# sizhe-li/neural-jacobian-field

Hardware: AMD Instinct MI355X
Metric: rendered rays/s (64 samples/ray, 256^2 image) (higher is better)
Workload: dtype f32 (v_mfma_f32_32x32x2_f32: exact fp32 products, fp32 accumulate -- the reference's arithmetic)

## Files before the change

neural-jacobian-field_amd/csrc/njf_device.h:

```cpp
#pragma once
#include <hip/hip_runtime.h>
#include <stdint.h>

__device__ __forceinline__ float relu_bits(float x) { return __int_as_float(max(__float_as_int(x), 0)); }

typedef float f32x16 __attribute__((ext_vector_type(16)));
typedef float f32x4 __attribute__((ext_vector_type(4)));
typedef _Float16 f16x8 __attribute__((ext_vector_type(8)));
typedef _Float16 f16x16 __attribute__((ext_vector_type(16)));
typedef _Float16 f16x32 __attribute__((ext_vector_type(32)));
typedef int i32x8 __attribute__((ext_vector_type(8)));
typedef int i32x4 __attribute__((ext_vector_type(4)));
typedef int i32x2 __attribute__((ext_vector_type(2)));
typedef unsigned u32x6 __attribute__((ext_vector_type(6)));

#define PREC_F32 0
#define PREC_F16X2 1
#define PREC_F16F6 2
#define PREC_F16 3

#define NJF_WAVES 4
#define NJF_THREADS (NJF_WAVES * 64)
#define NJF_CHUNK 8192

#define NJF_STREAM_BUFFERS 2
#define LDS_CTR_FLOATS 0
#define LDS_W0 0
#define LDS_W1 NJF_CHUNK
#define LDS_BIAS (NJF_STREAM_BUFFERS * NJF_CHUNK)
#define LDS_BIAS_FLOATS 2752
#define LDS_BIAS_FLOATS_PROPOSAL 1344
#define LDS_SCRATCH_PER_WAVE 528
#define LDS_FLOATS_RENDER (LDS_BIAS + LDS_BIAS_FLOATS + LDS_CTR_FLOATS)
#define LDS_FLOATS_PROPOSAL (LDS_BIAS + LDS_BIAS_FLOATS_PROPOSAL + NJF_WAVES * LDS_SCRATCH_PER_WAVE + LDS_CTR_FLOATS)
#define LDS_SCRATCH_PROPOSAL (LDS_BIAS + LDS_BIAS_FLOATS_PROPOSAL)

extern __shared__ __attribute__((aligned(16))) float njf_lds[];

__device__ __forceinline__ float mfma_step(float a, float b, f32x16& c) {
  c = __builtin_amdgcn_mfma_f32_32x32x2f32(a, b, c, 0, 0, 0);
  return 0.f;
}

#ifdef NJF_STAMPS
#define NJF_STAMP_SLOTS 1024
#ifdef NJF_STAMPS_PROPOSAL
#define NJF_STAMP_BASE LDS_FLOATS_PROPOSAL
#define NJF_STAMP_LOGS_PROPOSAL true
#else
#define NJF_STAMP_BASE LDS_FLOATS_RENDER
#define NJF_STAMP_LOGS_PROPOSAL false
#endif
__device__ unsigned njf_stamp_out[NJF_STAMP_SLOTS];
#define NJF_STAMP_FIELD int stamp_i;
#define NJF_STAMP_INIT(st) (st).stamp_i = -1
#define NJF_STAMP(st, tag)                                                                                   \
  do {                                                                                                       \
    if ((st).stamp_i >= 0 && (st).stamp_i < NJF_STAMP_SLOTS) {                                               \
      njf_lds[NJF_STAMP_BASE + (st).stamp_i] =                                                               \
          __uint_as_float(((unsigned)(tag) << 24) | ((unsigned)__builtin_readcyclecounter() & 0xffffffu));   \
      (st).stamp_i += 1;                                                                                     \
    }                                                                                                        \
  } while (0)
#define NJF_STAMP_P(st, tag) do { if (NJF_STAMP_LOGS_PROPOSAL) NJF_STAMP(st, tag); } while (0)
#define NJF_STAMP_ARM(st, IS_PROPOSAL, wave)                                                                                \
  const bool njf_stamping = ((IS_PROPOSAL) == NJF_STAMP_LOGS_PROPOSAL) && blockIdx.x == gridDim.x / 2 + 3 && (wave) == 1; \
  if (njf_stamping) (st).stamp_i = 0;                                                                                     \
  NJF_STAMP(st, 9)
#define NJF_STAMP_FLUSH(st, tag, lane)                                                                       \
  do {                                                                                                       \
    NJF_STAMP(st, tag);                                                                                      \
    if (njf_stamping)                                                                                        \
      for (int i_ = (lane); i_ < NJF_STAMP_SLOTS; i_ += 64)                                                  \
        njf_stamp_out[i_] = i_ < (st).stamp_i ? __float_as_uint(njf_lds[NJF_STAMP_BASE + i_]) : 0u;          \
  } while (0)
#define NJF_STAMP_PIN(...) asm volatile("" : __VA_ARGS__)
#define NJF_STAMP_LDS_FLOATS NJF_STAMP_SLOTS
#else
#define NJF_STAMP_FIELD
#define NJF_STAMP_INIT(st) do {} while (0)
#define NJF_STAMP(st, tag) do {} while (0)
#define NJF_STAMP_P(st, tag) do {} while (0)
#define NJF_STAMP_ARM(st, IS_PROPOSAL, wave) do {} while (0)
#define NJF_STAMP_FLUSH(st, tag, lane) do {} while (0)
#define NJF_STAMP_PIN(...) do {} while (0)
#define NJF_STAMP_LDS_FLOATS 0
#endif

struct WeightStreamState {
  __amdgpu_buffer_rsrc_t rsrc;
  int per_pass;
  int total;
  int idx;
  int in_pass;
  int dma_voff;
  int dma_soff;
  float* dma_dst;
  int dma_next;
  NJF_STAMP_FIELD
};
template <int GAP_AT_, int GAP_>
struct WeightStreamT : WeightStreamState {
  static constexpr int GAP_AT = GAP_AT_, GAP = GAP_;
};
typedef WeightStreamT<0x7fffffff, 0> WeightStream;
#define NJF_DMA_ROUNDS (NJF_CHUNK / (NJF_THREADS * 4))

__device__ __forceinline__ void dma_issue(const WeightStreamState& st, int r) {
#ifdef NJF_ABLATE_DMA
  return;
#endif
  __builtin_amdgcn_raw_ptr_buffer_load_lds(st.rsrc, (__attribute__((address_space(3))) void*)(st.dma_dst + r * NJF_THREADS * 4),
                                           16, st.dma_voff, st.dma_soff + r * NJF_THREADS * 16, 0, 0);
}

__device__ __forceinline__ void stream_flush(WeightStreamState& st) {
  if (st.dma_next == 0) {
#pragma unroll
    for (int r = 0; r < NJF_DMA_ROUNDS; ++r) dma_issue(st, r);
    st.dma_next = NJF_DMA_ROUNDS;
  }
}

template <class ST>
__device__ __forceinline__ void dma_job(ST& st, int chunk, int buf, int wave) {
  if constexpr (ST::GAP != 0) {
    if (chunk >= ST::GAP_AT) chunk += ST::GAP;
  }
  st.dma_soff = chunk * (NJF_CHUNK * 4) + wave * 1024;
  st.dma_dst = njf_lds + buf * NJF_CHUNK + wave * 256;
  st.dma_next = 0;
}

template <class ST>
__device__ __forceinline__ void stream_begin(ST& st, const float* g, int per_pass, int passes, int wave,
                                             int lane) {
  st.rsrc = __builtin_amdgcn_make_buffer_rsrc((void*)g, 0, 0x7ffffff0, 0x00020000);
  st.per_pass = per_pass;
  st.total = per_pass * passes;
  st.idx = 0;
  st.in_pass = 0;
  st.dma_voff = lane * 16;
  NJF_STAMP_INIT(st);
  dma_job(st, 0, 0, wave);
  stream_flush(st);
}

template <class ST>
__device__ __forceinline__ const float* stream_step(ST& st, int wave, int lane) {
#ifdef NJF_ABLATE_BARRIER
  return njf_lds + (st.idx++ & 1) * NJF_CHUNK;
#endif
  stream_flush(st);
  NJF_STAMP(st, 1);
  asm volatile("s_waitcnt vmcnt(0)" ::: "memory");
  NJF_STAMP(st, 2);
  __syncthreads();
  NJF_STAMP(st, 3);
  const float* cur = njf_lds + (st.idx & 1) * NJF_CHUNK;
  st.idx += 1;
  st.in_pass += 1;
  if (st.in_pass == st.per_pass) st.in_pass = 0;
  if (st.idx < st.total) dma_job(st, st.in_pass, st.idx & 1, wave);
  return cur;
}


typedef _Float16 f16x2 __attribute__((ext_vector_type(2)));
typedef unsigned u32x4 __attribute__((ext_vector_type(4)));
template <bool RELU>
__device__ __forceinline__ void split_pair(float x0, float x1, int p, f16x8& hi, f16x8& lo) {
  if (RELU) {
    x0 = relu_bits(x0);
    x1 = relu_bits(x1);
  }
  const _Float16 h0 = (_Float16)x0, h1 = (_Float16)x1;
  hi[2 * p] = h0;
  hi[2 * p + 1] = h1;
  const f16x2 hp = {h0, h1};
  const unsigned hu = __builtin_bit_cast(unsigned, hp);
  unsigned lu;
  asm("v_fma_mixlo_f16 %0, -%1, 1.0, %2 op_sel:[0,0,0] op_sel_hi:[1,0,0]" : "=v"(lu) : "v"(hu), "v"(x0));
  asm("v_fma_mixhi_f16 %0, -%1, 1.0, %2 op_sel:[1,0,0] op_sel_hi:[1,0,0]" : "+v"(lu) : "v"(hu), "v"(x1));
  u32x4 lv = __builtin_bit_cast(u32x4, lo);
  lv[p] = lu;
  lo = __builtin_bit_cast(f16x8, lv);
}

typedef unsigned u32x16 __attribute__((ext_vector_type(16)));
__device__ __forceinline__ unsigned pk_max_u16(unsigned a, unsigned b) {
  unsigned r;
  asm("v_pk_max_u16 %0, %1, %2" : "=v"(r) : "v"(a), "v"(b));
  return r;
}
template <bool RELU>
__device__ __forceinline__ void split_pair_u(float x0, float x1, unsigned& hu, unsigned& lu) {
  if (RELU) {
    x0 = relu_bits(x0);
    x1 = relu_bits(x1);
  }
  const f16x2 hp = {(_Float16)x0, (_Float16)x1};
  hu = __builtin_bit_cast(unsigned, hp);
  asm("v_fma_mixlo_f16 %0, -%1, 1.0, %2 op_sel:[0,0,0] op_sel_hi:[1,0,0]" : "=v"(lu) : "v"(hu), "v"(x0));
  asm("v_fma_mixhi_f16 %0, -%1, 1.0, %2 op_sel:[1,0,0] op_sel_hi:[1,0,0]" : "+v"(lu) : "v"(hu), "v"(x1));
}

typedef short s16x2 __attribute__((ext_vector_type(2)));
template <bool RELU>
__device__ __forceinline__ unsigned pack_pair_f16(float x0, float x1) {
  typedef float f32x2 __attribute__((ext_vector_type(2)));
  const f32x2 xp = {x0, x1};
  const f16x2 hp = __builtin_convertvector(xp, f16x2);
  if constexpr (RELU) {
    const s16x2 z = {0, 0};
    return __builtin_bit_cast(unsigned, __builtin_elementwise_max(__builtin_bit_cast(s16x2, hp), z));
  } else {
    return __builtin_bit_cast(unsigned, hp);
  }
}

#define F6_HI 0
#define F6_P1 16384
#define F6_P2 24576
#define F6_SCALE 28672


template <int PREC, int MBO, int NKB, int KB0, bool RELU, int KBI, class ST>
__device__ __forceinline__ void mma_chunk(ST& st, const float* __restrict__ wl, int lane,
                                          const f32x16 (&in)[KBI], f32x16 (&out)[MBO]) {
  constexpr bool SPREAD = MBO == 4 && (NKB == 2 || (PREC == PREC_F16 && NKB == 4)) && NJF_DMA_ROUNDS == 8;
  if constexpr (!SPREAD) stream_flush(st);
  if constexpr (PREC == PREC_F32) {
    const float* base = wl + lane * 4;
#pragma unroll
    for (int kb = 0; kb < NKB; ++kb) {
#pragma unroll
      for (int q = 0; q < 4; ++q) {
        f32x4 a[MBO];
#pragma unroll
        for (int m = 0; m < MBO; ++m) a[m] = *(const f32x4*)(base + ((kb * 4 + q) * MBO + m) * 256);
        if constexpr (SPREAD) {
          if (kb * 4 + q < 4) {
            dma_issue(st, 2 * (kb * 4 + q));
            dma_issue(st, 2 * (kb * 4 + q) + 1);
          }
        }
#pragma unroll
        for (int e = 0; e < 4; ++e) {
          float b = in[KB0 + kb][q * 4 + e];
          if (RELU) b = relu_bits(b);
#pragma unroll
          for (int m = 0; m < MBO; ++m) out[m] = __builtin_amdgcn_mfma_f32_32x32x2f32(a[m][e], b, out[m], 0, 0, 0);
        }
      }
    }
  } else if constexpr (PREC == PREC_F16F6 && MBO == 4 && NKB == 2) {
    typedef __attribute__((address_space(3))) const char* lds_ptr;
    const lds_ptr wb = (lds_ptr)(const char*)wl;
    lds_ptr p16 = wb + lane * 16;
    lds_ptr p8 = wb + lane * 8;
    asm volatile("" : "+v"(p16), "+v"(p8));
    unsigned bh[4][4], bl[4][4], mx[4];
#pragma unroll
    for (int p = 0; p < 4; ++p) {
      split_pair_u<RELU>(in[KB0][2 * p], in[KB0][2 * p + 1], bh[0][p], bl[0][p]);
      mx[p] = RELU ? bh[0][p] : (bh[0][p] & 0x7fff7fffu);
    }
#define NJF_LDS(T) const __attribute__((address_space(3))) T*
    auto hfrag = [&](int i) { return *(NJF_LDS(f16x8))(p16 + i * 1024); };
    auto f6frag = [&](int idx) {
      const i32x4 a4 = *(NJF_LDS(i32x4))(p16 + F6_P1 + idx * 1024);
      const i32x2 b2 = *(volatile NJF_LDS(i32x2))(p8 + F6_P2 + idx * 512);
      return i32x8{a4[0], a4[1], a4[2], a4[3], b2[0], b2[1], 0, 0};
    };
    auto op8 = [](const unsigned (&v)[4]) { return __builtin_bit_cast(f16x8, u32x4{v[0], v[1], v[2], v[3]}); };
    f16x8 a[2] = {hfrag(0), hfrag(1)};
    unsigned sb_h = 0, sb_l = 0;
    i32x8 bh6 = {0, 0, 0, 0, 0, 0, 0, 0}, wl6_0 = bh6, wl6_1 = bh6;
#pragma unroll
    for (int t = 0; t < 4; ++t) {
#pragma unroll
      for (int half = 0; half < 2; ++half) {
        const int u = 2 * t + half;
        f16x8 n[2] = {a[0], a[1]};
        if (u + 1 < 8) {
          n[0] = hfrag((u + 1) * 2);
          n[1] = hfrag((u + 1) * 2 + 1);
        } else {
          wl6_0 = f6frag(1);
          wl6_1 = f6frag(3);
        }
        if constexpr (SPREAD) {
          if (u < 4) {
            dma_issue(st, 2 * u);
            dma_issue(st, 2 * u + 1);
          }
        }
        __builtin_amdgcn_sched_barrier(0);
#pragma unroll
        for (int mm = 0; mm < 2; ++mm) {
          const int m = 2 * half + mm;
#ifdef NJF_ABLATE_MFMA
          asm volatile("" :: "v"(a[mm]), "v"(op8(bh[t])));
#else
          out[m] = __builtin_amdgcn_mfma_f32_32x32x16_f16(a[mm], op8(bh[t]), out[m], 0, 0, 0);
#endif
          if (t + 1 < 4) {
            const int kb2 = (t + 1) >> 1, tt2 = (t + 1) & 1;
            split_pair_u<RELU>(in[KB0 + kb2][8 * tt2 + 2 * m], in[KB0 + kb2][8 * tt2 + 2 * m + 1], bh[t + 1][m], bl[t + 1][m]);
            mx[m] = pk_max_u16(mx[m], RELU ? bh[t + 1][m] : (bh[t + 1][m] & 0x7fff7fffu));
          }
        }
        if (u == 6) {
          unsigned m2 = pk_max_u16(pk_max_u16(mx[0], mx[1]), pk_max_u16(mx[2], mx[3]));
          m2 = max(m2 & 0xffffu, m2 >> 16);
          const unsigned e5 = m2 >> 10;
          sb_h = e5 + 110u;
          sb_l = e5 + 99u;
          const u32x16 hv = {bh[0][0], bh[0][1], bh[0][2], bh[0][3], bh[1][0], bh[1][1], bh[1][2], bh[1][3],
                             bh[2][0], bh[2][1], bh[2][2], bh[2][3], bh[3][0], bh[3][1], bh[3][2], bh[3][3]};
          const u32x6 x6 = __builtin_amdgcn_cvt_scalef32_pk32_fp6_f16(__builtin_bit_cast(f16x32, hv), __uint_as_float(sb_h << 23));
          bh6 = i32x8{(int)x6[0], (int)x6[1], (int)x6[2], (int)x6[3], (int)x6[4], (int)x6[5], 0, 0};
        }
        a[0] = n[0];
        a[1] = n[1];
      }
    }
    const unsigned s_w0 = *(NJF_LDS(unsigned))(p8 + F6_SCALE - lane * 4);
    const unsigned s_w1 = *(NJF_LDS(unsigned))(p8 + F6_SCALE + 256 - lane * 4);
#undef NJF_LDS
    i32x8 wl6_2 = f6frag(5), wl6_3 = f6frag(7);
    __builtin_amdgcn_sched_barrier(0);
#ifdef NJF_ABLATE_MFMA
#define NJF_MFMA6(o, a6, b6, sel, sa, sb) asm volatile("" :: "v"(a6), "v"(b6), "v"(sa), "v"(sb))
#else
#define NJF_MFMA6(o, a6, b6, sel, sa, sb) o = __builtin_amdgcn_mfma_scale_f32_32x32x64_f8f6f4(a6, b6, o, 2, 2, sel, (int)(sa), 0, (int)(sb))
#endif
    NJF_MFMA6(out[0], wl6_0, bh6, 0, s_w1, sb_h);
    NJF_MFMA6(out[1], wl6_1, bh6, 1, s_w1, sb_h);
    i32x8 wh6_0 = f6frag(0), wh6_1 = f6frag(2);
    const u32x16 lv = {bl[0][0], bl[0][1], bl[0][2], bl[0][3], bl[1][0], bl[1][1], bl[1][2], bl[1][3],
                       bl[2][0], bl[2][1], bl[2][2], bl[2][3], bl[3][0], bl[3][1], bl[3][2], bl[3][3]};
    const u32x6 y6 = __builtin_amdgcn_cvt_scalef32_pk32_fp6_f16(__builtin_bit_cast(f16x32, lv), __uint_as_float(sb_l << 23));
    const i32x8 bl6 = {(int)y6[0], (int)y6[1], (int)y6[2], (int)y6[3], (int)y6[4], (int)y6[5], 0, 0};
    __builtin_amdgcn_sched_barrier(0);
    NJF_MFMA6(out[2], wl6_2, bh6, 2, s_w1, sb_h);
    NJF_MFMA6(out[3], wl6_3, bh6, 3, s_w1, sb_h);
    i32x8 wh6_2 = f6frag(4), wh6_3 = f6frag(6);
    __builtin_amdgcn_sched_barrier(0);
    NJF_MFMA6(out[0], wh6_0, bl6, 0, s_w0, sb_l);
    NJF_MFMA6(out[1], wh6_1, bl6, 1, s_w0, sb_l);
    NJF_MFMA6(out[2], wh6_2, bl6, 2, s_w0, sb_l);
    NJF_MFMA6(out[3], wh6_3, bl6, 3, s_w0, sb_l);
#undef NJF_MFMA6
    __builtin_amdgcn_sched_barrier(0);
  } else if constexpr (PREC == PREC_F16) {
    const f16x8* base = (const f16x8*)wl + lane;
    constexpr int T = NKB * 2;
    unsigned bc[4], bn[4];
#pragma unroll
    for (int p = 0; p < 4; ++p) bc[p] = pack_pair_f16<RELU>(in[KB0][2 * p], in[KB0][2 * p + 1]);
    auto op8 = [](const unsigned (&v)[4]) { return __builtin_bit_cast(f16x8, u32x4{v[0], v[1], v[2], v[3]}); };
    if constexpr (MBO == 4) {
      f16x8 a[4];
#pragma unroll
      for (int i = 0; i < 4; ++i) a[i] = base[i * 64];
#pragma unroll
      for (int t = 0; t < T; ++t) {
        f16x8 n[4] = {a[0], a[1], a[2], a[3]};
        if (t + 1 < T) {
#pragma unroll
          for (int i = 0; i < 4; ++i) n[i] = base[((t + 1) * 4 + i) * 64];
        }
        if constexpr (SPREAD) {
          if (t < 4) {
            dma_issue(st, 2 * t);
            dma_issue(st, 2 * t + 1);
          }
        }
        __builtin_amdgcn_sched_barrier(0);
#pragma unroll
        for (int m = 0; m < 4; ++m) {
#ifdef NJF_ABLATE_MFMA
          asm volatile("" :: "v"(a[m]), "v"(op8(bc)));
#else
          out[m] = __builtin_amdgcn_mfma_f32_32x32x16_f16(a[m], op8(bc), out[m], 0, 0, 0);
#endif
          if (t + 1 < T) {
            const int kb2 = (t + 1) >> 1, tt2 = (t + 1) & 1;
            bn[m] = pack_pair_f16<RELU>(in[KB0 + kb2][8 * tt2 + 2 * m], in[KB0 + kb2][8 * tt2 + 2 * m + 1]);
          }
        }
#pragma unroll
        for (int i = 0; i < 4; ++i) {
          a[i] = n[i];
          bc[i] = bn[i];
        }
      }
    } else {
#pragma unroll
      for (int t = 0; t < T; ++t) {
        f16x8 a[MBO];
#pragma unroll
        for (int m = 0; m < MBO; ++m) a[m] = base[(t * MBO + m) * 64];
        if (t + 1 < T) {
          const int kb2 = (t + 1) >> 1, tt2 = (t + 1) & 1;
#pragma unroll
          for (int p = 0; p < 4; ++p) bn[p] = pack_pair_f16<RELU>(in[KB0 + kb2][8 * tt2 + 2 * p], in[KB0 + kb2][8 * tt2 + 2 * p + 1]);
        }
#pragma unroll
        for (int m = 0; m < MBO; ++m) out[m] = __builtin_amdgcn_mfma_f32_32x32x16_f16(a[m], op8(bc), out[m], 0, 0, 0);
#pragma unroll
        for (int p = 0; p < 4; ++p) bc[p] = bn[p];
      }
    }
  } else {
    const f16x8* base = (const f16x8*)wl + lane;
    constexpr int T = NKB * 2;
    f16x8 bh, bl;
#pragma unroll
    for (int p = 0; p < 4; ++p) split_pair<RELU>(in[KB0][2 * p], in[KB0][2 * p + 1], p, bh, bl);
    if constexpr (MBO == 4) {
      f16x8 a[4];
#pragma unroll
      for (int i = 0; i < 4; ++i) a[i] = base[i * 64];
#pragma unroll
      for (int t = 0; t < T; ++t) {
        f16x8 nh = bh, nl = bl;
#pragma unroll
        for (int half = 0; half < 2; ++half) {
          const int u = 2 * t + half;
          f16x8 n[4] = {a[0], a[1], a[2], a[3]};
          if (u + 1 < 2 * T) {
#pragma unroll
            for (int i = 0; i < 4; ++i) n[i] = base[((u + 1) * 4 + i) * 64];
          }
          if constexpr (SPREAD) {
            if (u < 4) {
              dma_issue(st, 2 * u);
              dma_issue(st, 2 * u + 1);
            }
          }
          __builtin_amdgcn_sched_barrier(0);
#pragma unroll
          for (int mm = 0; mm < 2; ++mm) {
            const int m = 2 * half + mm;
#ifdef NJF_ABLATE_MFMA
            asm volatile("" :: "v"(a[2 * mm]), "v"(a[2 * mm + 1]), "v"(bh), "v"(bl));
#else
            out[m] = __builtin_amdgcn_mfma_f32_32x32x16_f16(a[2 * mm + 1], bh, out[m], 0, 0, 0);
            out[m] = __builtin_amdgcn_mfma_f32_32x32x16_f16(a[2 * mm], bl, out[m], 0, 0, 0);
            out[m] = __builtin_amdgcn_mfma_f32_32x32x16_f16(a[2 * mm], bh, out[m], 0, 0, 0);
#endif
            if (t + 1 < T) {
              const int kb2 = (t + 1) >> 1, tt2 = (t + 1) & 1;
              split_pair<RELU>(in[KB0 + kb2][8 * tt2 + 2 * m], in[KB0 + kb2][8 * tt2 + 2 * m + 1], m, nh, nl);
            }
          }
#pragma unroll
          for (int i = 0; i < 4; ++i) a[i] = n[i];
        }
        bh = nh;
        bl = nl;
      }
    } else {
#pragma unroll
      for (int t = 0; t < T; ++t) {
        f16x8 ah[MBO], al[MBO];
#pragma unroll
        for (int m = 0; m < MBO; ++m) {
          ah[m] = base[((t * MBO + m) * 2 + 0) * 64];
          al[m] = base[((t * MBO + m) * 2 + 1) * 64];
        }
        f16x8 nh = bh, nl = bl;
        if (t + 1 < T) {
          const int kb2 = (t + 1) >> 1, tt2 = (t + 1) & 1;
#pragma unroll
          for (int p = 0; p < 4; ++p)
            split_pair<RELU>(in[KB0 + kb2][8 * tt2 + 2 * p], in[KB0 + kb2][8 * tt2 + 2 * p + 1], p, nh, nl);
        }
#pragma unroll
        for (int m = 0; m < MBO; ++m) {
          out[m] = __builtin_amdgcn_mfma_f32_32x32x16_f16(al[m], bh, out[m], 0, 0, 0);
          out[m] = __builtin_amdgcn_mfma_f32_32x32x16_f16(ah[m], bl, out[m], 0, 0, 0);
          out[m] = __builtin_amdgcn_mfma_f32_32x32x16_f16(ah[m], bh, out[m], 0, 0, 0);
        }
        bh = nh;
        bl = nl;
      }
    }
  }
  if constexpr (SPREAD) st.dma_next = NJF_DMA_ROUNDS;
}

template <int MB, bool ASSIGN, int PREC = PREC_F16F6, bool SPLIT = false>
__device__ __forceinline__ void bias_init(const float* __restrict__ bl, int hh, f32x16 (&acc)[MB]) {
#ifdef NJF_ABLATE_BIAS
  if (ASSIGN)
    for (int m = 0; m < MB; ++m) acc[m] = (f32x16)(0.f);
  return;
#endif
  constexpr bool VALU = ASSIGN || (PREC != PREC_F16F6 && PREC != PREC_F16);
  if constexpr (!ASSIGN && PREC == PREC_F16 && SPLIT) {
    const int i = threadIdx.x & 31;
    const float* b = bl + 16 * MB * ((i >> 2) & 1) + 4 * (i >> 3) + (i & 3);
    const f16x8 ones = __builtin_bit_cast(f16x8, u32x4{hh == 0 ? 0x3c003c00u : 0u, 0u, 0u, 0u});
#pragma unroll
    for (int m = 0; m < MB; ++m) {
      const unsigned u = hh == 0 ? __float_as_uint(b[16 * m]) : 0u;
      acc[m] = __builtin_amdgcn_mfma_f32_32x32x16_f16(__builtin_bit_cast(f16x8, u32x4{u, 0u, 0u, 0u}), ones, acc[m], 0, 0, 0);
    }
  } else if constexpr (VALU) {
    const float* b = bl + 16 * MB * hh;
#pragma unroll
    for (int m = 0; m < MB; ++m) {
#pragma unroll
      for (int q = 0; q < 4; ++q) {
        f32x4 v = *(const f32x4*)(b + 16 * m + 4 * q);
#pragma unroll
        for (int e = 0; e < 4; ++e) {
          if (ASSIGN) acc[m][4 * q + e] = v[e];
          else acc[m][4 * q + e] += v[e];
        }
      }
    }
  } else {
    const int i = threadIdx.x & 31;
    const float one = hh == 0 ? 1.f : 0.f;
    const float* b = bl + 16 * MB * ((i >> 2) & 1) + 4 * (i >> 3) + (i & 3);
#pragma unroll
    for (int m = 0; m < MB; ++m) {
      const float a = b[16 * m];
      if (ASSIGN) acc[m] = __builtin_amdgcn_mfma_f32_32x32x2f32(a, one, (f32x16)(0.f), 0, 0, 0);
      else acc[m] = __builtin_amdgcn_mfma_f32_32x32x2f32(a, one, acc[m], 0, 0, 0);
    }
  }
}

struct CamCtx;
struct PointGeom {
  float xc, yc, zc;
  const CamCtx* cam;
  int hf, wf, stride;
  unsigned gofs;
};
struct Footprint {
  int t00, t01, t10, t11;
  float w00, w01, w10, w11;
};

struct CamCtx {
  float m[12];
  float k[9];
};

__device__ __forceinline__ void load_ctx(const float* __restrict__ w2c, const float* __restrict__ k, int b,
                                         CamCtx& c) {
#pragma unroll
  for (int i = 0; i < 12; ++i) c.m[i] = w2c[b * 16 + i];
#pragma unroll
  for (int i = 0; i < 9; ++i) c.k[i] = k[b * 9 + i];
}

__device__ __forceinline__ float dot4_h(const float* r, float x, float y, float z) {
  float a = r[0] * x;
  a = fmaf(r[1], y, a);
  a = fmaf(r[2], z, a);
  a = fmaf(r[3], 1.0f, a);
  return a;
}

__device__ __forceinline__ float dot3(const float* r, float x, float y, float z) {
  float a = r[0] * x;
  a = fmaf(r[1], y, a);
  a = fmaf(r[2], z, a);
  return a;
}

__device__ __forceinline__ void point_geometry(const CamCtx& c, float px, float py, float pz, int hf, int wf,
                                               int stride, unsigned gofs, PointGeom& g) {
  g.gofs = gofs;
  g.xc = dot4_h(c.m + 0, px, py, pz);
  g.yc = dot4_h(c.m + 4, px, py, pz);
  g.zc = dot4_h(c.m + 8, px, py, pz);
  g.cam = &c;
  g.hf = hf;
  g.wf = wf;
  g.stride = stride;
}

__device__ __forceinline__ void point_footprint(const PointGeom& g, Footprint& f) {
  float xc = g.xc, yc = g.yc, zc = g.zc;
  asm volatile("" : "+v"(xc), "+v"(yc), "+v"(zc));
  const CamCtx& c = *g.cam;
  const int hf = g.hf, wf = g.wf, stride = g.stride;
  const float u0 = dot3(c.k + 0, xc, yc, zc);
  const float u1 = dot3(c.k + 3, xc, yc, zc);
  const float u2 = dot3(c.k + 6, xc, yc, zc);
  const float den = u2 + 1e-9f;
  const float inv = __builtin_amdgcn_rcpf(den);
  const float u = u0 * inv, v = u1 * inv;
  const float gx = (u - 0.5f) * 2.0f, gy = (v - 0.5f) * 2.0f;
  float ix = ((gx + 1.0f) / 2.0f) * (float)(wf - 1);
  float iy = ((gy + 1.0f) / 2.0f) * (float)(hf - 1);
  ix = fminf((float)(wf - 1), fmaxf(ix, 0.0f));
  iy = fminf((float)(hf - 1), fmaxf(iy, 0.0f));
  const float x0f = floorf(ix), y0f = floorf(iy);
  const float fx = ix - x0f, fy = iy - y0f;
  const float ex = 1.0f - fx, ey = 1.0f - fy;
  int x0 = (int)x0f, y0 = (int)y0f;
  x0 = min(max(x0, 0), wf - 1);
  y0 = min(max(y0, 0), hf - 1);
  const int x1 = min(x0 + 1, wf - 1), y1 = min(y0 + 1, hf - 1);
  f.t00 = (y0 * wf + x0) * stride;
  f.t01 = (y0 * wf + x1) * stride;
  f.t10 = (y1 * wf + x0) * stride;
  f.t11 = (y1 * wf + x1) * stride;
  f.w00 = ey * ex;
  f.w01 = ey * fx;
  f.w10 = fy * ex;
  f.w11 = fy * fx;
}

template <int S>
__device__ __forceinline__ unsigned quad_bcast(unsigned v) {
  return (unsigned)__builtin_amdgcn_update_dpp(0, (int)v, S | (S << 2) | (S << 4) | (S << 6), 0xf, 0xf, true);
}
__device__ __forceinline__ unsigned quad_bcast_n(unsigned v, int s) {
  return s == 0 ? quad_bcast<0>(v) : (s == 1 ? quad_bcast<1>(v) : (s == 2 ? quad_bcast<2>(v) : quad_bcast<3>(v)));
}

template <int MB, int DEPTH = 4>
__device__ __forceinline__ void add_hoisted_latent_quad(const float* __restrict__ gz, const PointGeom& g, int lane,
                                                        f32x16 (&h)[MB]) {
#ifdef NJF_ABLATE_GATHER
  return;
#endif
  Footprint f;
  point_footprint(g, f);
  const int c = lane & 3;
  const unsigned lane_off = 16 * MB * (lane >> 5) + 4 * c;
  const unsigned gofs = g.gofs;
  const unsigned own[4] = {gofs + (unsigned)f.t00, gofs + (unsigned)f.t01, gofs + (unsigned)f.t10, gofs + (unsigned)f.t11};
  const float w[4] = {f.w00, f.w01, f.w10, f.w11};
  f32x4 x[DEPTH][MB];
  auto issue = [&](int b) {
    const float* src = gz + (size_t)(quad_bcast_n(own[b >> 2], b & 3) + lane_off);
#pragma unroll
    for (int m = 0; m < MB; ++m) x[b % DEPTH][m] = *(const f32x4*)(src + 16 * m);
  };
#pragma unroll
  for (int b = 0; b < DEPTH; ++b) issue(b);
#pragma unroll
  for (int b = 0; b < 16; ++b) {
    const float wb = c == (b & 3) ? w[b >> 2] : 0.f;
#pragma unroll
    for (int m = 0; m < MB; ++m)
#pragma unroll
      for (int e = 0; e < 4; ++e) {
        f32x4 d = {h[m][4 * e], h[m][4 * e + 1], h[m][4 * e + 2], h[m][4 * e + 3]};
        d = __builtin_amdgcn_mfma_f32_4x4x1f32(x[b % DEPTH][m][e], wb, d, 0, 0, 0);
        h[m][4 * e] = d[0];
        h[m][4 * e + 1] = d[1];
        h[m][4 * e + 2] = d[2];
        h[m][4 * e + 3] = d[3];
      }
    if (b + DEPTH < 16) issue(b + DEPTH);
    __builtin_amdgcn_sched_barrier(0);
  }
}


template <int MB, int DEPTH = 4>
__device__ __forceinline__ void add_hoisted_latent_half(const float* __restrict__ gz, const PointGeom& g, int hh,
                                                        f32x16 (&h)[MB]) {
#ifdef NJF_ABLATE_GATHER
  return;
#endif
  Footprint f;
  point_footprint(g, f);
  const float* gb = gz + (size_t)g.gofs + 4 * hh;
  const float* p[4] = {gb + f.t00, gb + f.t01, gb + f.t10, gb + f.t11};
  const float w[4] = {f.w00, f.w01, f.w10, f.w11};
  constexpr int NB = 4 * MB;
  f32x4 v[DEPTH][4];
  auto issue = [&](int b) {
    const float* src = p[b / MB] + 32 * (b % MB);
#pragma unroll
    for (int q = 0; q < 4; ++q) v[b % DEPTH][q] = *(const f32x4*)(src + 8 * q);
  };
#pragma unroll
  for (int b = 0; b < DEPTH; ++b) issue(b);
#pragma unroll
  for (int b = 0; b < NB; ++b) {
    const int t = b / MB, m = b % MB;
#pragma unroll
    for (int q = 0; q < 4; ++q)
#pragma unroll
      for (int e = 0; e < 4; ++e) {
        if (t == 0) {
          h[m][4 * q + e] = fmaf(v[b % DEPTH][q][e], w[0], h[m][4 * q + e]);
        } else {
          float acc = h[m][4 * q + e];
          asm("v_fmac_f32 %0, %1, %2" : "+v"(acc) : "v"(v[b % DEPTH][q][e]), "v"(w[t]));
          h[m][4 * q + e] = acc;
        }
      }
    asm volatile("" : "+v"(h[m]) : : "memory");
    if (b + DEPTH < NB) issue(b + DEPTH);
    __builtin_amdgcn_sched_barrier(0);
  }
}

#define NJF_F16_GATHER_DEPTH 8
template <int MB, int DEPTH = NJF_F16_GATHER_DEPTH>
__device__ __forceinline__ void add_hoisted_latent_f16(const _Float16* __restrict__ gz, const PointGeom& g, int hh,
                                                       f32x16 (&h)[MB], const Footprint* shared = nullptr) {
#ifdef NJF_ABLATE_GATHER
  return;
#endif
  Footprint f;
  if (shared != nullptr) f = *shared;
  else point_footprint(g, f);
  const _Float16* gb = gz + (size_t)g.gofs + 8 * hh;
  const _Float16* p[4] = {gb + f.t00, gb + f.t01, gb + f.t10, gb + f.t11};
  const float w[4] = {f.w00, f.w01, f.w10, f.w11};
  constexpr int NB = 4 * MB;
  constexpr int D = DEPTH < NB ? DEPTH : NB;
  f16x8 v[D][2];
  auto issue = [&](int b) {
    const _Float16* src = p[b / MB] + 32 * (b % MB);
#pragma unroll
    for (int q = 0; q < 2; ++q) v[b % D][q] = *(const f16x8*)(src + 16 * q);
  };
#pragma unroll
  for (int b = 0; b < D; ++b) issue(b);
#pragma unroll
  for (int b = 0; b < NB; ++b) {
    const int t = b / MB, m = b % MB;
#pragma unroll
    for (int q = 0; q < 2; ++q)
#pragma unroll
      for (int e = 0; e < 8; ++e) h[m][8 * q + e] = fmaf((float)v[b % D][q][e], w[t], h[m][8 * q + e]);
    asm volatile("" : "+v"(h[m]) : : "memory");
    if (b + D < NB) issue(b + D);
    __builtin_amdgcn_sched_barrier(0);
  }
}

struct TileShareF16 {
  unsigned pe[16];
};

__device__ __forceinline__ void share_tile(const f32x16 (&pe)[2], TileShareF16& sh) {
#pragma unroll
  for (int t = 0; t < 4; ++t)
#pragma unroll
    for (int p = 0; p < 4; ++p) sh.pe[4 * t + p] = pack_pair_f16<false>(pe[t >> 1][8 * (t & 1) + 2 * p], pe[t >> 1][8 * (t & 1) + 2 * p + 1]);
}

template <class ST>
__device__ __forceinline__ void mma_lin_in_f16_packed(ST& st, const float* __restrict__ wl, int lane, const unsigned (&pk)[16],
                                                      f32x16 (&out)[4]) {
  const f16x8* base = (const f16x8*)wl + lane;
  constexpr int T = 4;
  f16x8 a[4];
#pragma unroll
  for (int i = 0; i < 4; ++i) a[i] = base[i * 64];
#pragma unroll
  for (int t = 0; t < T; ++t) {
    f16x8 n[4] = {a[0], a[1], a[2], a[3]};
    if (t + 1 < T) {
#pragma unroll
      for (int i = 0; i < 4; ++i) n[i] = base[((t + 1) * 4 + i) * 64];
    }
    dma_issue(st, 2 * t);
    dma_issue(st, 2 * t + 1);
    __builtin_amdgcn_sched_barrier(0);
    const f16x8 b = __builtin_bit_cast(f16x8, u32x4{pk[4 * t], pk[4 * t + 1], pk[4 * t + 2], pk[4 * t + 3]});
#pragma unroll
    for (int m = 0; m < 4; ++m) out[m] = __builtin_amdgcn_mfma_f32_32x32x16_f16(a[m], b, out[m], 0, 0, 0);
#pragma unroll
    for (int i = 0; i < 4; ++i) a[i] = n[i];
  }
}


template <int MB, int PREC, int DEPTH = 4>
__device__ __forceinline__ void add_hoisted_latent(const float* __restrict__ gz, const PointGeom& g, int lane,
                                                   f32x16 (&h)[MB]) {
  if constexpr (PREC == PREC_F16) add_hoisted_latent_f16<MB>((const _Float16*)gz, g, lane >> 5, h);
  else if constexpr (PREC == PREC_F16F6) add_hoisted_latent_quad<MB, DEPTH>(gz, g, lane, h);
  else add_hoisted_latent_half<MB, DEPTH>(gz, g, lane >> 5, h);
}

template <int PREC>
__device__ __forceinline__ const float* map_at(const float* base, size_t elements) {
  if constexpr (PREC == PREC_F16) return (const float*)((const _Float16*)base + elements);
  else return base + elements;
}

__device__ __forceinline__ float sin_accurate(float arg) {
  const float C_HI = 0.15915493667125702f, C_LO = 6.4206382432985265e-09f;
  const float u = arg * C_HI;
  float e = fmaf(arg, C_HI, -u);
  e = fmaf(arg, C_LO, e);
  const float y = (u - rintf(u)) + e;
  return __builtin_amdgcn_sinf(y);
}

__device__ __forceinline__ void positional_encoding(float xc, float yc, float zc, int hh, f32x16 (&pe)[2]) {
#ifdef NJF_ABLATE_PE
  pe[0] = (f32x16)(xc);
  pe[1] = (f32x16)(yc + zc);
  return;
#endif
  const float two_pi = 6.2831855f;
  const float half_pi = hh ? 1.5707964f : 0.0f;
  const float sx[3] = {two_pi * xc, two_pi * yc, two_pi * zc};
#pragma unroll
  for (int s = 0; s < 30; ++s) {
    const int d = s / 10, f = s % 10;
    const float arg = sx[d] * (float)(1 << f) + half_pi;
    pe[s >> 4][s & 15] = sin_accurate(arg);
  }
  pe[1][14] = hh ? zc : xc;
  pe[1][15] = hh ? 1.0f : yc;
}

__device__ __forceinline__ void sh4(float dx, float dy, float dz, float (&o)[16]) {
  const float x = ((dx + 1.0f) / 2.0f) * 2.0f - 1.0f;
  const float y = ((dy + 1.0f) / 2.0f) * 2.0f - 1.0f;
  const float z = ((dz + 1.0f) / 2.0f) * 2.0f - 1.0f;
  const float xy = x * y, xz = x * z, yz = y * z, x2 = x * x, y2 = y * y, z2 = z * z;
  o[0] = 0.28209479177387814f;
  o[1] = -0.48860251190291987f * y;
  o[2] = 0.48860251190291987f * z;
  o[3] = -0.48860251190291987f * x;
  o[4] = 1.0925484305920792f * xy;
  o[5] = -1.0925484305920792f * yz;
  o[6] = 0.94617469575755997f * z2 - 0.31539156525251999f;
  o[7] = -1.0925484305920792f * xz;
  o[8] = 0.54627421529603959f * x2 - 0.54627421529603959f * y2;
  o[9] = 0.59004358992664352f * y * (-3.0f * x2 + y2);
  o[10] = 2.8906114426405538f * xy * z;
  o[11] = 0.45704579946446572f * y * (1.0f - 5.0f * z2);
  o[12] = 0.3731763325901154f * z * (5.0f * z2 - 3.0f);
  o[13] = 0.45704579946446572f * x * (1.0f - 5.0f * z2);
  o[14] = 1.4453057213202769f * z * (x2 - y2);
  o[15] = 0.59004358992664352f * x * (-x2 + 3.0f * y2);
}

struct ActDump {
  float* act;
  float* pe;
  size_t stride;
  unsigned* mask = nullptr;
  bool half = false;
  float* feat = nullptr;
};

__device__ __forceinline__ float* dump_layer(const ActDump& d, int l) {
  if (d.act == nullptr) return nullptr;
  return d.half ? (float*)((_Float16*)d.act + (size_t)l * d.stride) : d.act + (size_t)l * d.stride;
}

template <bool DO_RELU>
__device__ __forceinline__ void dump_vec128(float* __restrict__ dst, const f32x16 (&v)[4], unsigned* __restrict__ mask = nullptr,
                                            bool half = false) {
  if (dst == nullptr) return;
  if (half) {
    _Float16* d16 = (_Float16*)dst;
#pragma unroll
    for (int m = 0; m < 4; ++m)
#pragma unroll
      for (int q = 0; q < 2; ++q) {
        u32x4 o;
#pragma unroll
        for (int e = 0; e < 4; ++e) o[e] = pack_pair_f16<DO_RELU>(v[m][8 * q + 2 * e], v[m][8 * q + 2 * e + 1]);
        *(u32x4*)(d16 + 16 * m + 8 * q) = o;
      }
  } else {
#pragma unroll
  for (int m = 0; m < 4; ++m)
#pragma unroll
    for (int q = 0; q < 4; ++q) {
      f32x4 o;
#pragma unroll
      for (int e = 0; e < 4; ++e) o[e] = DO_RELU ? fmaxf(v[m][4 * q + e], 0.f) : v[m][4 * q + e];
      *(f32x4*)(dst + 16 * m + 4 * q) = o;
    }
  }
  if (mask != nullptr) {
    unsigned w[2] = {0u, 0u};
#pragma unroll
    for (int m = 0; m < 4; ++m)
#pragma unroll
      for (int r = 0; r < 16; ++r) {
        const unsigned b = (unsigned)min(max(__float_as_int(v[m][r]), 0), 1);
        w[m >> 1] |= b << (16 * (m & 1) + r);
      }
    typedef unsigned u32x2 __attribute__((ext_vector_type(2)));
    *(u32x2*)mask = u32x2{w[0], w[1]};
  }
}

template <int PREC, bool DUMP = false, int SHARED = 0, class ST>
__device__ __forceinline__ void resnet_tile(ST& st, const float* __restrict__ bias,
                                            const float* __restrict__ gz, const PointGeom& g,
                                            const f32x16 (&pe)[2], int wave, int lane, f32x16 (&out)[1],
                                            ActDump dump = ActDump{nullptr, nullptr, 0}, const TileShareF16* share = nullptr) {
  static_assert(SHARED == 0 || (PREC == PREC_F16 && !DUMP), "the shared tile state exists for the plain-fp16 inference kernels");
  const int hh = lane >> 5;
  f32x16 h[4], net[4];
#pragma unroll
  for (int m = 0; m < 4; ++m) h[m] = (f32x16)(0.f);
  if (DUMP && dump.pe != nullptr) {
#pragma unroll
    for (int kb = 0; kb < 2; ++kb)
#pragma unroll
      for (int q = 0; q < 4; ++q) {
        f32x4 o;
#pragma unroll
        for (int e = 0; e < 4; ++e) o[e] = pe[kb][4 * q + e];
        *(f32x4*)(dump.pe + 16 * kb + 4 * q) = o;
      }
  }
  {
    const float* wl = stream_step(st, wave, lane);
    if constexpr ((SHARED & 1) != 0) mma_lin_in_f16_packed(st, wl, lane, share->pe, h);
    else mma_chunk<PREC, 4, 2, 0, false, 2>(st, wl, lane, pe, h);
  }
  if constexpr (PREC == PREC_F16) {
    static_assert(!DUMP, "the plain-fp16 mode is an inference mode (training forwards dump fp32-class activations)");
    Footprint fp_net;
    if constexpr ((SHARED & 2) != 0) point_footprint(g, fp_net);
    for (int blk = 0; blk < 5; ++blk) {
      if (blk < 3) {
        NJF_STAMP(st, 4);
        if constexpr ((SHARED & 2) != 0) add_hoisted_latent_f16<4>((const _Float16*)map_at<PREC>(gz, blk * 128), g, hh, h, &fp_net);
        else add_hoisted_latent<4, PREC>(map_at<PREC>(gz, blk * 128), g, lane, h);
        NJF_STAMP(st, 5);
      }
      const float* bl = bias + blk * 256;
      bias_init<4, true, PREC>(bl, hh, net);
      {
        const float* wl = stream_step(st, wave, lane);
        mma_chunk<PREC, 4, 4, 0, true, 4>(st, wl, lane, h, net);
      }
      if (blk >= 2) bias_init<4, false, PREC, true>(bl + 128, hh, h);
      {
        const float* wl = stream_step(st, wave, lane);
        mma_chunk<PREC, 4, 4, 0, true, 4>(st, wl, lane, net, h);
      }
    }
  } else
  for (int blk = 0; blk < 5; ++blk) {
    if (blk < 3) {
      NJF_STAMP(st, 4);
      add_hoisted_latent<4, PREC>(gz + blk * 128, g, lane, h);
      NJF_STAMP(st, 5);
    }
    if (DUMP) dump_vec128<true>(dump_layer(dump, 2 * blk), h, dump.mask ? dump.mask + (size_t)(2 * blk) * (dump.stride / 32) : nullptr, dump.half);
    const float* bl = bias + blk * 256;
    bias_init<4, true, PREC>(bl, hh, net);
    {
      {
        const float* wl = stream_step(st, wave, lane);
        mma_chunk<PREC, 4, 2, 0, true, 4>(st, wl, lane, h, net);
      }
      {
        const float* wl = stream_step(st, wave, lane);
        mma_chunk<PREC, 4, 2, 2, true, 4>(st, wl, lane, h, net);
      }
    }
    if (DUMP) dump_vec128<true>(dump_layer(dump, 2 * blk + 1), net, dump.mask ? dump.mask + (size_t)(2 * blk + 1) * (dump.stride / 32) : nullptr, dump.half);
    bias_init<4, false, PREC>(bl + 128, hh, h);
    {
      {
        const float* wl = stream_step(st, wave, lane);
        mma_chunk<PREC, 4, 2, 0, true, 4>(st, wl, lane, net, h);
      }
      {
        const float* wl = stream_step(st, wave, lane);
        mma_chunk<PREC, 4, 2, 2, true, 4>(st, wl, lane, net, h);
      }
    }
    if (DUMP && dump.feat != nullptr) dump_vec128<false>(dump.feat + (size_t)blk * dump.stride, h);
  }
  if (DUMP) dump_vec128<true>(dump_layer(dump, 10), h, dump.mask ? dump.mask + (size_t)10 * (dump.stride / 32) : nullptr, dump.half);
  bias_init<1, true, PREC>(bias + 1280, hh, out);
  {
    const float* wl = stream_step(st, wave, lane);
    mma_chunk<PREC, 1, 4, 0, true, 4>(st, wl, lane, h, out);
  }
}

struct ColorDump {
  float* in;
  float* act;
  size_t stride;
};

template <bool DO_RELU>
__device__ __forceinline__ void dump_vec32(float* __restrict__ dst, const f32x16 (&v)[2]) {
#pragma unroll
  for (int m = 0; m < 2; ++m)
#pragma unroll
    for (int q = 0; q < 4; ++q) {
      f32x4 o;
#pragma unroll
      for (int e = 0; e < 4; ++e) o[e] = DO_RELU ? fmaxf(v[m][4 * q + e], 0.f) : v[m][4 * q + e];
      *(f32x4*)(dst + 16 * m + 4 * q) = o;
    }
}

template <int PREC, bool DUMP = false, class ST>
__device__ __forceinline__ void color_tile(ST& st, const float* __restrict__ bias, const f32x16 (&cin)[1],
                                           int wave, int lane, f32x16 (&rgb)[1],
                                           ColorDump dump = ColorDump{nullptr, nullptr, 0}) {
  const int hh = lane >> 5;
  const float* wl = stream_step(st, wave, lane);
  f32x16 a[2], b[2];
  a[0] = (f32x16)(0.f);
  a[1] = (f32x16)(0.f);
  mma_chunk<PREC, 2, 1, 0, false, 1>(st, wl, lane, cin, a);
  bias_init<2, true, PREC>(bias, hh, b);
  mma_chunk<PREC, 2, 2, 0, true, 2>(st, wl + 2048, lane, a, b);
  bias_init<1, true, PREC>(bias + 64, hh, rgb);
  mma_chunk<PREC, 1, 2, 0, true, 2>(st, wl + 6144, lane, b, rgb);
  if (DUMP && dump.in != nullptr) {
#pragma unroll
    for (int q = 0; q < 4; ++q) {
      f32x4 o;
#pragma unroll
      for (int e = 0; e < 4; ++e) o[e] = cin[0][4 * q + e];
      *(f32x4*)(dump.in + 4 * q) = o;
    }
    dump_vec32<true>(dump.act, a);
    dump_vec32<true>(dump.act + dump.stride, b);
  }
}

__device__ __forceinline__ float erf_branchless(float a) {
  const float t = fabsf(a), s = a * a;
  float r = fmaf(-1.72853470e-5f, t, 3.83197126e-4f);
  const float u = fmaf(-3.88396438e-3f, t, 2.42546219e-2f);
  r = fmaf(r, s, u);
  r = fmaf(r, t, -1.06777877e-1f);
  r = fmaf(r, t, -6.34846687e-1f);
  r = fmaf(r, t, -1.28717512e-1f);
  r = fmaf(r, t, -t);
  const float hi = copysignf(1.0f - __builtin_amdgcn_exp2f(r * 1.4426950408889634f), a);
  float q = -5.96761703e-4f;
  q = fmaf(q, s, 4.99119423e-3f);
  q = fmaf(q, s, -2.67681349e-2f);
  q = fmaf(q, s, 1.12819925e-1f);
  q = fmaf(q, s, -3.76125336e-1f);
  q = fmaf(q, s, 1.28379166e-1f);
  const float lo = fmaf(q, a, a);
  return t > 0.927734375f ? hi : lo;
}

__device__ __forceinline__ float erf_as7126(float a) {
  const float t = __builtin_amdgcn_rcpf(fmaf(0.3275911f, fabsf(a), 1.0f));
  float p = 1.061405429f;
  p = fmaf(p, t, -1.453152027f);
  p = fmaf(p, t, 1.421413741f);
  p = fmaf(p, t, -0.284496736f);
  p = fmaf(p, t, 0.254829592f);
  p *= t;
  const float e = __builtin_amdgcn_exp2f((a * a) * -1.4426950408889634f);
  return copysignf(fmaf(-p, e, 1.0f), a);
}

__device__ __forceinline__ void norm64(const f32x16 (&x)[2], f32x16 (&n)[2]) {
  float s = 0.f;
#pragma unroll
  for (int m = 0; m < 2; ++m)
#pragma unroll
    for (int r = 0; r < 16; ++r) s += x[m][r];
  s += __shfl_xor(s, 32, 64);
  const float mean = s / 64.0f;
  float v = 0.f;
#pragma unroll
  for (int m = 0; m < 2; ++m)
#pragma unroll
    for (int r = 0; r < 16; ++r) {
      const float d = x[m][r] - mean;
      v = fmaf(d, d, v);
    }
  v += __shfl_xor(v, 32, 64);
  const float rstd = __builtin_amdgcn_rsqf(v / 64.0f + 1e-5f);
  const float shift = -mean * rstd;
#pragma unroll
  for (int m = 0; m < 2; ++m)
#pragma unroll
    for (int r = 0; r < 16; ++r) n[m][r] = fmaf(x[m][r], rstd, shift);
}

__device__ __forceinline__ void store_vec64(float* __restrict__ dst, const f32x16 (&v)[2]) {
  if (dst == nullptr) return;
#pragma unroll
  for (int m = 0; m < 2; ++m)
#pragma unroll
    for (int q = 0; q < 4; ++q) {
      f32x4 o;
#pragma unroll
      for (int e = 0; e < 4; ++e) o[e] = v[m][4 * q + e];
      *(f32x4*)(dst + 16 * m + 4 * q) = o;
    }
}
__device__ __forceinline__ void load_vec64(const float* __restrict__ src, bool ok, f32x16 (&v)[2]) {
#pragma unroll
  for (int m = 0; m < 2; ++m)
#pragma unroll
    for (int q = 0; q < 4; ++q) {
      f32x4 o = {0.f, 0.f, 0.f, 0.f};
      if (ok) o = *(const f32x4*)(src + 16 * m + 4 * q);
#pragma unroll
      for (int e = 0; e < 4; ++e) v[m][4 * q + e] = o[e];
    }
}

template <int PREC, class ST>
__device__ __forceinline__ void transformer_tile(ST& st, const float* __restrict__ bias,
                                                 const float* __restrict__ gq, const PointGeom& g,
                                                 const f32x16 (&pe)[2], int keys, int wave, int lane, f32x16 (&out)[1],
                                                 float* __restrict__ xdump = nullptr, size_t xstride = 0) {
  const int hh = lane >> 5;
  f32x16 x[2], n[2], t[2];
  x[0] = (f32x16)(0.f);
  x[1] = (f32x16)(0.f);
  const float* wl = stream_step(st, wave, lane);
  mma_chunk<PREC, 2, 2, 0, false, 2>(st, wl, lane, pe, x);
  add_hoisted_latent<2, PREC>(gq, g, lane, x);
  for (int l = 0; l < 3; ++l) {
    const float* bl = bias + 256 * l;
    if (xdump != nullptr) store_vec64(xdump + (size_t)l * xstride, x);
    norm64(x, n);
    bias_init<2, true, PREC>(bl, hh, t);
    mma_chunk<PREC, 2, 2, 0, false, 2>(st, wl + 4096, lane, n, t);
#pragma unroll
    for (int m = 0; m < 2; ++m) {
#pragma unroll
      for (int h8 = 0; h8 < 2; ++h8) {
        float mx = -3.0e38f;
#pragma unroll
        for (int a = 0; a < 8; ++a)
          if (a < keys) mx = fmaxf(mx, t[m][8 * h8 + a]);
        float e[8], sum = 0.f;
#pragma unroll
        for (int a = 0; a < 8; ++a) {
          e[a] = (a < keys) ? __builtin_amdgcn_exp2f((t[m][8 * h8 + a] - mx) * 1.4426950408889634f) : 0.f;
          sum += e[a];
        }
        const float inv = __builtin_amdgcn_rcpf(sum);
#pragma unroll
        for (int a = 0; a < 8; ++a) t[m][8 * h8 + a] = e[a] * inv;
      }
    }
    wl = stream_step(st, wave, lane);
    bias_init<2, false, PREC>(bl + 64, hh, x);
    mma_chunk<PREC, 2, 2, 0, false, 2>(st, wl, lane, t, x);
    norm64(x, n);
    bias_init<2, true, PREC>(bl + 128, hh, t);
    mma_chunk<PREC, 2, 2, 0, false, 2>(st, wl + 4096, lane, n, t);
#pragma unroll
    for (int m = 0; m < 2; ++m)
#pragma unroll
      for (int r = 0; r < 16; ++r) {
        const float v = t[m][r];
        const float z = v * 0.70710678118654752440f;
        const float ef = PREC == PREC_F32 ? erf_branchless(z) : erf_as7126(z);
        t[m][r] = 0.5f * v * (1.0f + ef);
      }
    wl = stream_step(st, wave, lane);
    bias_init<2, false, PREC>(bl + 192, hh, x);
    mma_chunk<PREC, 2, 2, 0, false, 2>(st, wl, lane, t, x);
  }
  if (xdump != nullptr) store_vec64(xdump + 3 * xstride, x);
  bias_init<1, true, PREC>(bias + 768, hh, out);
  mma_chunk<PREC, 1, 2, 0, false, 2>(st, wl + 4096, lane, x, out);
}

__device__ __forceinline__ float norm64_rstd(const f32x16 (&x)[2], f32x16 (&n)[2]) {
  float s = 0.f;
#pragma unroll
  for (int m = 0; m < 2; ++m)
#pragma unroll
    for (int r = 0; r < 16; ++r) s += x[m][r];
  s += __shfl_xor(s, 32, 64);
  const float mean = s / 64.0f;
  float v = 0.f;
#pragma unroll
  for (int m = 0; m < 2; ++m)
#pragma unroll
    for (int r = 0; r < 16; ++r) {
      const float d = x[m][r] - mean;
      v = fmaf(d, d, v);
    }
  v += __shfl_xor(v, 32, 64);
  const float rstd = __builtin_amdgcn_rsqf(v / 64.0f + 1e-5f);
  const float shift = -mean * rstd;
#pragma unroll
  for (int m = 0; m < 2; ++m)
#pragma unroll
    for (int r = 0; r < 16; ++r) n[m][r] = fmaf(x[m][r], rstd, shift);
  return rstd;
}
__device__ __forceinline__ void norm64_backward(const f32x16 (&dn)[2], const f32x16 (&n)[2], float rstd, f32x16 (&acc)[2]) {
  float s0 = 0.f, s1 = 0.f;
#pragma unroll
  for (int m = 0; m < 2; ++m)
#pragma unroll
    for (int r = 0; r < 16; ++r) {
      s0 += dn[m][r];
      s1 = fmaf(dn[m][r], n[m][r], s1);
    }
  s0 += __shfl_xor(s0, 32, 64);
  s1 += __shfl_xor(s1, 32, 64);
  const float m0 = s0 / 64.0f, m1 = s1 / 64.0f;
#pragma unroll
  for (int m = 0; m < 2; ++m)
#pragma unroll
    for (int r = 0; r < 16; ++r) acc[m][r] = fmaf(rstd, dn[m][r] - m0 - n[m][r] * m1, acc[m][r]);
}

__device__ __forceinline__ float half_sum(float v) {
#pragma unroll
  for (int o = 16; o >= 1; o >>= 1) v += __shfl_xor(v, o, 64);
  return v;
}
__device__ __forceinline__ float half_min(float v) {
#pragma unroll
  for (int o = 16; o >= 1; o >>= 1) v = fminf(v, __shfl_xor(v, o, 64));
  return v;
}
__device__ __forceinline__ float half_max(float v) {
#pragma unroll
  for (int o = 16; o >= 1; o >>= 1) v = fmaxf(v, __shfl_xor(v, o, 64));
  return v;
}
__device__ __forceinline__ float half_scan(float v, int j) {
#pragma unroll
  for (int o = 1; o < 32; o <<= 1) {
    const float t = __shfl_up(v, o, 32);
    if (j >= o) v += t;
  }
  return v;
}

__device__ __forceinline__ int xcd_remap(int bid, int nwg) {
  const int q = nwg >> 3, r = nwg & 7, xcd = bid & 7, i = bid >> 3;
  return (xcd < r ? xcd * (q + 1) : r * (q + 1) + (xcd - r) * q) + i;
}
```

Baseline: 1.963 million.

## Interleave latent bilinear gather with fp32 MFMA chunks in the MLP

Adds a fused fp32 routine that issues the latent-grid bilinear gather loads and folds them into the output accumulators while the preceding layer's 32x32x2 MFMAs for the next block run, instead of doing the gather as a separate phase. It is used for the input layer and the last chunk of blocks 0 and 1 in the fp32 non-dump path, hiding gather memory latency behind matrix work. The fold schedule is hand-spread across MFMA slots, and DMA rounds are issued inside the routine. This raises register pressure and ties the code to a fixed DMA round count.

```diff
diff --git a/neural-jacobian-field_amd/csrc/njf_device.h b/neural-jacobian-field_amd/csrc/njf_device.h
--- a/neural-jacobian-field_amd/csrc/njf_device.h
+++ b/neural-jacobian-field_amd/csrc/njf_device.h
@@ -622,6 +622,11 @@
   f.w11 = fy * fx;
 }
 
+#ifdef NJF_ABLATE_GATHER
+#define NJF_GATHER false
+#else
+#define NJF_GATHER true
+#endif
 template <int S>
 __device__ __forceinline__ unsigned quad_bcast(unsigned v) {
   return (unsigned)__builtin_amdgcn_update_dpp(0, (int)v, S | (S << 2) | (S << 4) | (S << 6), 0xf, 0xf, true);
@@ -633,9 +638,7 @@
 template <int MB, int DEPTH = 4>
 __device__ __forceinline__ void add_hoisted_latent_quad(const float* __restrict__ gz, const PointGeom& g, int lane,
                                                         f32x16 (&h)[MB]) {
-#ifdef NJF_ABLATE_GATHER
-  return;
-#endif
+  if (!NJF_GATHER) return;
   Footprint f;
   point_footprint(g, f);
   const int c = lane & 3;
@@ -674,9 +677,7 @@
 template <int MB, int DEPTH = 4>
 __device__ __forceinline__ void add_hoisted_latent_half(const float* __restrict__ gz, const PointGeom& g, int hh,
                                                         f32x16 (&h)[MB]) {
-#ifdef NJF_ABLATE_GATHER
-  return;
-#endif
+  if (!NJF_GATHER) return;
   Footprint f;
   point_footprint(g, f);
   const float* gb = gz + (size_t)g.gofs + 4 * hh;
@@ -716,9 +717,7 @@
 template <int MB, int DEPTH = NJF_F16_GATHER_DEPTH>
 __device__ __forceinline__ void add_hoisted_latent_f16(const _Float16* __restrict__ gz, const PointGeom& g, int hh,
                                                        f32x16 (&h)[MB], const Footprint* shared = nullptr) {
-#ifdef NJF_ABLATE_GATHER
-  return;
-#endif
+  if (!NJF_GATHER) return;
   Footprint f;
   if (shared != nullptr) f = *shared;
   else point_footprint(g, f);
@@ -851,6 +850,88 @@
   o[15] = 0.59004358992664352f * x * (-x2 + 3.0f * y2);
 }
 
+template <int KB0, bool RELU, int KBI, class ST>
+__device__ __forceinline__ void mma_chunk_gather_f32(ST& st, const float* __restrict__ wl, int lane, const f32x16 (&in)[KBI],
+                                                     f32x16 (&out)[4], const float* __restrict__ gz, const PointGeom& g) {
+  static_assert(NJF_DMA_ROUNDS == 8, "one DMA round behind every second group of blocks 0 and 1");
+  constexpr int DEPTH = 2;
+  constexpr int FIRST = 4;
+  Footprint f;
+  point_footprint(g, f);
+  const float* gb = gz + (size_t)g.gofs + 4 * (lane >> 5);
+  const float* p[4] = {gb + f.t00, gb + f.t01, gb + f.t10, gb + f.t11};
+  const float w[4] = {f.w00, f.w01, f.w10, f.w11};
+  f32x4 v[DEPTH][4];
+  auto issue = [&](int b) {
+    const float* src = p[b & 3] + 32 * (b >> 2);
+#pragma unroll
+    for (int q = 0; q < 4; ++q) v[b % DEPTH][q] = *(const f32x4*)(src + 8 * q);
+  };
+  auto fold = [&](int m, int i) {
+    const int t = i >> 4, r = i & 15, b = 4 * m + t;
+    if (t == 0) {
+      out[m][r] = fmaf(v[b % DEPTH][r >> 2][r & 3], w[0], out[m][r]);
+    } else {
+      float acc = out[m][r];
+      asm("v_fmac_f32 %0, %1, %2" : "+v"(acc) : "v"(v[b % DEPTH][r >> 2][r & 3]), "v"(w[t]));
+      out[m][r] = acc;
+    }
+  };
+  auto refill = [&](int m, int t) {
+    asm volatile("" : "+v"(out[m]) : : "memory");
+    if (4 * m + t + DEPTH < 16) issue(4 * m + t + DEPTH);
+  };
+  auto folded = [](int n) { return n <= FIRST ? 0 : (n - FIRST) * 64 / (32 - FIRST); };
+  if (NJF_GATHER) {
+#pragma unroll
+    for (int b = 0; b < DEPTH; ++b) issue(b);
+  }
+  const float* base = wl + lane * 4;
+  f32x16 bin[2];
+  f32x4 a = *(const f32x4*)base;
+#pragma unroll
+  for (int m = 0; m < 4; ++m) {
+#pragma unroll
+    for (int kq = 0; kq < 8; ++kq) {
+      const int kb = kq >> 2, q = kq & 3, gi = 8 * m + kq;
+      f32x4 n = a;
+      if (gi + 1 < 32) n = *(const f32x4*)(base + (((gi + 1) & 7) * 4 + ((gi + 1) >> 3)) * 256);
+      if (gi < 16 && (gi & 1) == 0) dma_issue(st, gi >> 1);
+#pragma unroll
+      for (int e = 0; e < 4; ++e) {
+        if (m == 0) {
+          float b = in[KB0 + kb][q * 4 + e];
+          if (RELU) b = relu_bits(b);
+          bin[kb][q * 4 + e] = b;
+        }
+        out[m] = __builtin_amdgcn_mfma_f32_32x32x2f32(a[e], bin[kb][q * 4 + e], out[m], 0, 0, 0);
+        if (NJF_GATHER && m > 0) {
+#pragma unroll
+          for (int i = folded(4 * kq + e); i < folded(4 * kq + e + 1); ++i) fold(m - 1, i);
+        }
+      }
+      if (NJF_GATHER && m > 0) {
+#pragma unroll
+        for (int t = folded(4 * kq) / 16; t < folded(4 * kq + 4) / 16; ++t) refill(m - 1, t);
+      }
+      a = n;
+      __builtin_amdgcn_sched_barrier(0);
+    }
+  }
+  st.dma_next = NJF_DMA_ROUNDS;
+  NJF_STAMP(st, 4);
+  if (NJF_GATHER) {
+#pragma unroll
+    for (int t = 0; t < 4; ++t) {
+#pragma unroll
+      for (int i = 16 * t; i < 16 * t + 16; ++i) fold(3, i);
+      refill(3, t);
+      __builtin_amdgcn_sched_barrier(0);
+    }
+  }
+  NJF_STAMP(st, 5);
+}
+
 struct ActDump {
   float* act;
   float* pe;
@@ -912,6 +993,7 @@
                                             ActDump dump = ActDump{nullptr, nullptr, 0}, const TileShareF16* share = nullptr) {
   static_assert(SHARED == 0 || (PREC == PREC_F16 && !DUMP), "the shared tile state exists for the plain-fp16 inference kernels");
   const int hh = lane >> 5;
+  constexpr bool FUSED = PREC == PREC_F32 && !DUMP;
   f32x16 h[4], net[4];
 #pragma unroll
   for (int m = 0; m < 4; ++m) h[m] = (f32x16)(0.f);
@@ -929,6 +1011,7 @@
   {
     const float* wl = stream_step(st, wave, lane);
     if constexpr ((SHARED & 1) != 0) mma_lin_in_f16_packed(st, wl, lane, share->pe, h);
+    else if constexpr (FUSED) mma_chunk_gather_f32<0, false, 2>(st, wl, lane, pe, h, gz, g);
     else mma_chunk<PREC, 4, 2, 0, false, 2>(st, wl, lane, pe, h);
   }
   if constexpr (PREC == PREC_F16) {
@@ -956,7 +1039,7 @@
     }
   } else
   for (int blk = 0; blk < 5; ++blk) {
-    if (blk < 3) {
+    if (!FUSED && blk < 3) {
       NJF_STAMP(st, 4);
       add_hoisted_latent<4, PREC>(gz + blk * 128, g, lane, h);
       NJF_STAMP(st, 5);
@@ -983,7 +1066,14 @@
       }
       {
         const float* wl = stream_step(st, wave, lane);
-        mma_chunk<PREC, 4, 2, 2, true, 4>(st, wl, lane, net, h);
+        bool plain = true;
+        if constexpr (FUSED) {
+          if (blk < 2) {
+            mma_chunk_gather_f32<2, true, 4>(st, wl, lane, net, h, gz + (blk + 1) * 128, g);
+            plain = false;
+          }
+        }
+        if (plain) mma_chunk<PREC, 4, 2, 2, true, 4>(st, wl, lane, net, h);
       }
     }
     if (DUMP && dump.feat != nullptr) dump_vec128<false>(dump.feat + (size_t)blk * dump.stride, h);
```

Result: faster. 2.022 million, median of 6 (+3.0%).
